# JuliaLinearAlgebra/RecursiveFactorization.jl

Hardware: AMD Instinct MI355X
Metric: LU GFLOP/s (2n^3/3) on NxN Float64, 1/2/4/8 MI355X; ||PA-LU||/||A|| (higher is better)
Workload: dtype f64; 1 GPU; lu!(A, ipiv) of a dense uniform[0,1) 16384x16384 Float64 matrix, partial pivoting, column-major in HBM; n=16384, pivot=True, blocksize=0, layout=single GPU

## Files before the change

recursivefactorization.jl_amd/build.py:

```python
from __future__ import annotations

import os
import subprocess
from concurrent.futures import ThreadPoolExecutor

HERE = os.path.dirname(os.path.abspath(__file__))
CSRC = os.path.join(HERE, "csrc")
OBJ = os.path.join(CSRC, "build_exp" if os.environ.get("RFLU_EXPERIMENTS", "0") not in ("", "0") else "build")
LIB = os.path.join(HERE, "librflu_exp.so" if os.environ.get("RFLU_EXPERIMENTS", "0") not in ("", "0") else "librflu.so")
EXPERIMENTS = os.environ.get("RFLU_EXPERIMENTS", "0") not in ("", "0")
SOURCES = ["gemm.hip", "engine.hip", "panel.hip", "panel_f32.hip", "panel_local.hip", "panel_local_f32.hip", "panel_local_xcd.hip", "panel_local_xcd_f32.hip", "panel_single.hip", "panel_single_f32.hip", "trsm.hip", "trsv.hip", "laswp.hip", "butterfly.hip", "driver.cpp"]
if EXPERIMENTS:
    SOURCES += ["panel_blocked.hip", "panel_blocked_f32.hip"]
HEADERS = ["rflu_internal.hpp", os.path.join("..", "..", "include", "rflu.h")]
ALL_HEADERS = HEADERS + ["panel_common.hpp", "panel_xchg.hpp", "trsm_row.hpp", "gemm_tile.hpp", "laswp_strip.hpp", "engine.hpp", "schedule_plan.hpp"]
_PANEL_H = ["panel_common.hpp", "panel_xchg.hpp", "trsm_row.hpp"]
EXTRA_DEPS = {"gemm.hip": ["gemm_tile.hpp"], "engine.hip": ["gemm_tile.hpp", "laswp_strip.hpp", "engine.hpp"], "driver.cpp": ["engine.hpp", "schedule_plan.hpp"],
              "laswp.hip": ["laswp_strip.hpp", "trsm_row.hpp"], "trsm.hip": ["trsm_row.hpp"], "trsv.hip": ["trsm_row.hpp"],
              "panel.hip": _PANEL_H, "panel_local.hip": _PANEL_H, "panel_single.hip": _PANEL_H, "panel_blocked.hip": _PANEL_H,
              "panel_f32.hip": ["panel.hip", *_PANEL_H], "panel_local_f32.hip": ["panel_local.hip", *_PANEL_H],
              "panel_local_xcd.hip": ["panel_local.hip", *_PANEL_H], "panel_local_xcd_f32.hip": ["panel_local.hip", *_PANEL_H],
              "panel_single_f32.hip": ["panel_single.hip", *_PANEL_H], "panel_blocked_f32.hip": ["panel_blocked.hip", *_PANEL_H]}
FLAGS = ["--offload-arch=gfx950", "-O3", "-std=c++17", "-fPIC", "-x", "hip", "-Wno-unused-result"] + (["-DRFLU_EXPERIMENTS"] if EXPERIMENTS else [])


def _mtime(p):
    return os.path.getmtime(p) if os.path.exists(p) else 0.0


def _digest(paths):
    import hashlib

    h = hashlib.sha1(" ".join(FLAGS).encode())
    for p in paths:
        with open(p, "rb") as f:
            h.update(f.read())
    return h.hexdigest()


def sources_digest() -> str:
# ... 56 lines not shown
```

recursivefactorization.jl_amd/csrc/driver.cpp:

```cpp
#include <stdarg.h>
#include <stdio.h>
#include <stdlib.h>
#include <string.h>

#include <algorithm>
#include <new>

#include "rflu_internal.hpp"
#include "engine.hpp"
#include "schedule_plan.hpp"
#include <atomic>
#include <chrono>
#include <thread>

namespace rflu {

static thread_local char g_err[512] = "";

void set_error(const char* fmt, ...)
{
    va_list ap;
    va_start(ap, fmt);
    vsnprintf(g_err, sizeof(g_err), fmt, ap);
    va_end(ap);
// ... 59 lines not shown
    env_get("RFLU_SPLIT_SHARE", split_share);
    env_get("RFLU_MAX_RESERVE", max_reserve);
    env_get("RFLU_WIDE_NARROW", wide_narrow);
    env_get("RFLU_NARROW_COLS", narrow_cols);
    env_get("RFLU_RESERVE_CUS", min_reserve);
    env_get("RFLU_CONFINE_ROWS", confine_rows);
    env_get("RFLU_MERGE_ROWS", merge_rows);
    env_get("RFLU_SWAP_SU", swap_su);
    env_get("RFLU_SWAP_LATE", swap_late);
    env_get("RFLU_SWAP_ROWS", swap_rows);
    env_get("RFLU_GATE_FOLD", gate_fold);
    env_flag("RFLU_TIME_ENQUEUE", time_enqueue);
    env_get("RFLU_TAIL_OVERLAP", tail_overlap);
    env_get("RFLU_MGPU_TALL_ROWS", mgpu_tall_rows);
    env_get("RFLU_MGPU_SYNC", mgpu_sync);
    env_get("RFLU_ENGINE_POLICY", engine_policy);
    env_get("RFLU_ENGINE_WGS", engine_wgs);
    env_get("RFLU_ENGINE_WC", engine_wc);
    env_get("RFLU_ENGINE_WRITE_THROUGH", engine_write_through);
    env_get("RFLU_ENGINE_LEAF_XCDS", engine_leaf_xcds);
    env_get("RFLU_ENGINE_LEAF_WGS", engine_leaf_wgs);
    env_get("RFLU_ENGINE_HOST_LAG", engine_host_lag);
    env_get("RFLU_ENGINE_SOLVE_RL", engine_solve_rl);
#endif
}

static void load_handle_env(Handle* h)
{
    h->tune.load_env();
    h->coop_launch = false;
    h->panel_local = 2;
    h->panel_single = 1;
    h->panel_blocked = 0;
    h->panel_local_maxg = 64;
    int v = 0;
    env_get("RFLU_COOP_LAUNCH", v);
    h->coop_launch = v != 0;
    env_get("RFLU_PANEL_LOCAL", h->panel_local);
    env_get("RFLU_PANEL_SINGLE", h->panel_single);
    env_get("RFLU_PANEL_BLOCKED", h->panel_blocked);
    if (h->panel_local == 1) h->panel_local_maxg = 32;
#ifdef RFLU_EXPERIMENTS
    env_get("RFLU_PANEL_LOCAL_MAXG", h->panel_local_maxg);
#endif
}

// ... 4 lines not shown
    if (pad > 0 && ld % 512 == 0) ld += pad;
    return ld;
}

int ensure_buffer(void** ptr, size_t* cap, size_t need)
{
    if (*cap >= need) return RFLU_OK;
    if (*ptr) RFLU_HIP(hipFree(*ptr));
    *ptr = nullptr;
    *cap = 0;
    RFLU_HIP(hipMalloc(ptr, need));
    *cap = need;
    return RFLU_OK;
}

int ensure_bookkeeping(Handle* h, int64_t rows)
{
    const int64_t chunks = (rows + NB - 1) / NB + 1;
    if (chunks <= h->pm_chunks) return RFLU_OK;
    if (h->pm_cnt) RFLU_HIP(hipFree(h->pm_cnt));
    if (h->pm_dst) RFLU_HIP(hipFree(h->pm_dst));
    if (h->pm_src) RFLU_HIP(hipFree(h->pm_src));
    if (h->linv) RFLU_HIP(hipFree(h->linv));
    h->linv = nullptr;
    h->pm_cnt = h->pm_dst = h->pm_src = nullptr;
    h->pm_chunks = 0;
    RFLU_HIP(hipMalloc((void**)&h->pm_cnt, (size_t)chunks * sizeof(int)));
    RFLU_HIP(hipMalloc((void**)&h->pm_dst, (size_t)chunks * 2 * NB * sizeof(int)));
    RFLU_HIP(hipMalloc((void**)&h->pm_src, (size_t)chunks * 2 * NB * sizeof(int)));
    RFLU_HIP(hipMalloc(&h->linv, (size_t)chunks * NB * NB * sizeof(double)));
    RFLU_HIP(hipMemset(h->pm_cnt, 0, (size_t)chunks * sizeof(int)));
    h->pm_chunks = chunks;
    return RFLU_OK;
}

constexpr int64_t TRSM_FUSED_MAX = 256;

template <typename T>
static int trsm_rec(Handle* h, int64_t n, int64_t nrhs, const T* L, int64_t ldl, T* B, int64_t ldb, const T* linv)
{
    if (n <= 0 || nrhs <= 0) return RFLU_OK;
    if (linv && n <= TRSM_FUSED_MAX) return launch_trsm_fused<T>(h, n, nrhs, L, ldl, linv, B, ldb);
    if (n <= NB) return launch_trsm_base<T>(h, n, nrhs, L, ldl, B, ldb);
    const int64_t leaves = (n + NB - 1) / NB;
    const int64_t n1 = ((leaves + 1) / 2) * NB;
    RFLU_TRY(trsm_rec<T>(h, n1, nrhs, L, ldl, B, ldb, linv));
    RFLU_TRY(launch_gemm<T>(h, n - n1, nrhs, n1, L + n1 * ldl, ldl, B, ldb, B + n1 * ldb, ldb));
    return trsm_rec<T>(h, n - n1, nrhs, L + n1 * ldl + n1, ldl, B + n1 * ldb, ldb,
                       linv ? linv + (n1 / NB) * NB * NB : nullptr);
}

template <typename T>
static int trsm_public(Handle* h, int64_t n, int64_t nrhs, const T* L, int64_t ldl, T* B, int64_t ldb)
{
// ... 676 lines not shown
            c.lclaim = lk < nleft ? (unsigned long long)lk << 32 : (unsigned long long)ENG_SEQ_DONE << 32;
            c.lprog = (unsigned long long)lk;
            if (nleft > 0 && lk > 0) img->cb[eng_first_cb(geo, eng_pb(geo, cb))].leftdone += 1ull << 32;
            img->remaining += lk < nleft;
        }
        if (h->tune.engine_replay) {
            if (eng_end < nblk) { set_error("RFLU_ENGINE_REPLAY needs the engine to the end"); return RFLU_ERR_ARG; }
            RFLU_TRY(launch_gate_signal(h, h->gate_ptr[0], val(nleaf - 1)));
            if (f.tail) { RFLU_HIP(hipStreamWaitEvent(P, f.tail, 0)); f.tail = nullptr; }
        }
        RFLU_HIP(hipMemcpyAsync(reinterpret_cast<char*>(est) + skip, reinterpret_cast<char*>(img) + skip, bytes - skip, hipMemcpyHostToDevice, P));
        RFLU_TRY(record_on(P, EX + (size_t)nblk + 1));
        RFLU_TRY(wait_on(E, EX + (size_t)nblk + 1));
        EngArgs<T> a;
        a.R = R; a.ld = ld; a.g = geo; a.policy = h->tune.engine_policy;
        a.linv = static_cast<const T*>(h->linv); a.pm_cnt = h->pm_cnt; a.pm_dst = h->pm_dst; a.pm_src = h->pm_src;
        a.st = est; a.leaf_gate = h->gate_ptr[0]; a.gate_base = gbase; a.info = h->info_dev; a.gemm_flags = h->tune.gemm_flags;
        a.arrived = h->eng_host_mode ? &est->arrived : nullptr;
        a.rows_final = h->eng_host_mode ? h->eng_rows_final_dev : nullptr;
        a.write_through = h->tune.engine_write_through != 0;
        a.leaf_xcds = h->tune.engine_leaf_xcds;
        a.leaf_wgs = h->tune.engine_leaf_wgs;
        a.solve_rl = h->tune.engine_solve_rl != 0;
        a.host_lag = h->eng_host_mode ? h->tune.engine_host_lag : 0;
        a.retire_xcc = -1; a.retire_leaf = 0;
        if (eng_retire_leaf >= 0) {
            a.retire_xcc = h->panel_xcc;
            a.retire_leaf = (int)std::max<int64_t>(1, eng_retire_leaf - 2);
        }
        a.trace = nullptr;
        long long*& eng_trace_buf = h->eng_trace_buf;
        if (env_str("RFLU_ENGINE_TRACE")) {
            if (!eng_trace_buf) RFLU_HIP(hipMalloc((void**)&eng_trace_buf, (4096 * 4 + 16) * sizeof(long long)));
            else {
                std::vector<long long> hs(4096 * 4 + 16);
                RFLU_HIP(hipMemcpy(hs.data(), eng_trace_buf, hs.size() * sizeof(long long), hipMemcpyDeviceToHost));
                double s01 = 0, s12 = 0, s23 = 0, sq = 0; int cnt = 0;
                for (int g = 1; g + 1 < (int)nleaf && g < 4095; ++g) {
                    if (!hs[g * 4] || !hs[g * 4 + 3] || !hs[(g - 1) * 4 + 3]) continue;
                    s01 += (hs[g * 4 + 1] - hs[g * 4]) / 100.0; s12 += (hs[g * 4 + 2] - hs[g * 4 + 1]) / 100.0; s23 += (hs[g * 4 + 3] - hs[g * 4 + 2]) / 100.0;
                    sq += (hs[g * 4] - hs[(g - 1) * 4 + 3]) / 100.0; ++cnt;
                }
                if (cnt) fprintf(stderr, "[rflu] engine trace (previous call, %d leaf windows on their first column block): first claim -> stage 0 done %.1f us, -> first tile claimed %.1f, -> window complete %.1f; previous window complete -> first claim %.1f us\n", cnt, s01 / cnt, s12 / cnt, s23 / cnt, sq / cnt);
                {
                    const long long* ac = hs.data() + 4096 * 4;
                    const double tot = (double)(ac[0] + ac[1] + ac[2] + ac[3] + ac[4]);
                    if (tot > 0)
                        fprintf(stderr, "[rflu] engine workgroup time (previous call, %.1f workgroup-ms): block-column tiles %.1f %%, leaf-window tiles %.1f %%, strips + solves %.1f %%, deferred interchanges %.1f %%, between units %.1f %% (of which asleep with nothing eligible %.1f %%, count + publication behind a unit %.1f %%, scan / claim / acquire %.1f %%)\n",
                                tot / 1e5, 100.0 * ac[0] / tot, 100.0 * ac[1] / tot, 100.0 * ac[2] / tot, 100.0 * ac[3] / tot, 100.0 * ac[4] / tot, 100.0 * ac[5] / tot, 100.0 * ac[6] / tot, 100.0 * (ac[4] - ac[5] - ac[6]) / tot);
                    if (tot > 0 && ac[15] > 0)
                        fprintf(stderr, "[rflu] engine scan (previous call, %lld calls, %.2f sweeps per call), us per call: epoch / gate sample %.2f, exit words %.2f, claim words + choice %.2f, ticket %.2f, "
                                        "scan of the deferred interchanges %.2f, acquire + hand-over %.2f; asleep %.2f\n",
                                ac[15], (double)ac[14] / ac[15], ac[8] / 100.0 / ac[15], ac[9] / 100.0 / ac[15], ac[10] / 100.0 / ac[15], ac[11] / 100.0 / ac[15], ac[12] / 100.0 / ac[15],
                                ac[13] / 100.0 / ac[15], ac[5] / 100.0 / ac[15]);
                }
                int tg0 = 40, tgn = 4;
                if (const char* e = env_str("RFLU_ENGINE_TRACE")) { if (strchr(e, ':')) sscanf(e, "%d:%d", &tg0, &tgn); }
                for (int g = std::max(tg0, 1); g < tg0 + tgn && g + 1 < (int)nleaf && g < 4095; ++g)
                {
                    fprintf(stderr, "   leaf %d: first claim at %.3f ms | stage 0 %.1f us | to first tile %.1f | tiles %.1f | idle before %.1f", g, (hs[g * 4] - hs[0]) / 1e5,
                            (hs[g * 4 + 1] - hs[g * 4]) / 100.0, (hs[g * 4 + 2] - hs[g * 4 + 1]) / 100.0, (hs[g * 4 + 3] - hs[g * 4 + 2]) / 100.0, (hs[g * 4] - hs[(g - 1) * 4 + 3]) / 100.0);
                    const long long* n4 = hs.data() + (size_t)(2048 + g) * 4;
                    if (g < 2048 && n4[0] && n4[3])
                        fprintf(stderr, " || next block column: first claim at %.3f ms (%.1f us after the previous leaf's window there was complete) | stage 0 %.1f | to first tile %.1f | tiles %.1f",
                                (n4[0] - hs[0]) / 1e5, (n4[0] - n4[-1]) / 100.0, (n4[1] - n4[0]) / 100.0, (n4[2] - n4[1]) / 100.0, (n4[3] - n4[2]) / 100.0);
                    fprintf(stderr, "\n");
                    const int LPBt = (int)(W / NB);
                    if ((g + 1) % LPBt == 0 && g / LPBt < 512) {
                        const int b = g / LPBt;
                        const long long* bg = hs.data() + (size_t)(1024 + b) * 4;
                        const long long* lf = hs.data() + (size_t)(1536 + b) * 4;
                        const long long t0 = n4[0];
                        if (t0 && bg[0] && bg[3])
                            fprintf(stderr, "   block column %d ends (its last leaf's window is claimed at +0): own deferred interchanges +%.0f .. +%.0f us | BIG(%d) on the first column block of block column %d: "
                                            "stage 0 +%.0f .. +%.0f | tiles +%.0f .. +%.0f us\n",
                                    b, (lf[0] - t0) / 100.0, (lf[1] - t0) / 100.0, b, b + 2, (bg[0] - t0) / 100.0, (bg[1] - t0) / 100.0, (bg[2] - t0) / 100.0, (bg[3] - t0) / 100.0);
                    }
                }
            }
            RFLU_HIP(hipMemsetAsync(eng_trace_buf, 0, (4096 * 4 + 16) * sizeof(long long), P));
            a.trace = eng_trace_buf;
        }
        const int wgs = h->tune.engine_wgs > 0 ? h->tune.engine_wgs : 2 * (h->num_cus - 32);
        if (img->remaining > 0) {
            double eng_flops = 0, eng_bytes = 0;
            for (int cb = 0; cb < geo.ncb; ++cb) {
                for (int k = 0; k < eng_nops(geo, cb); ++k) {
                    const EngOp o = eng_op(geo, cb, k);
                    if (o.nc <= 0) continue;
                    const double M = (double)std::max(geo.m - (o.j0 + o.jb), 0), N = (double)o.nc, K = (double)o.jb;
                    eng_flops += 2.0 * M * N * K;
                    eng_bytes += sizeof(T) * (M * K + K * N + 2.0 * M * N + 2.0 * K * N + 0.5 * K * K + (f.pivot ? 4.0 * K * N : 0.0));
                }
                if (f.pivot && eng_pb(geo, cb) < geo.nbp) {
                    const double nc = (double)(std::min<int64_t>(n, (int64_t)(cb + 1) * geo.Wc) - (int64_t)cb * geo.Wc);
                    const double later = (double)std::max<int64_t>(std::min<int64_t>((int64_t)geo.nbp * W, mn) - (int64_t)(eng_pb(geo, cb) + 1) * W, 0);
                    eng_bytes += sizeof(T) * 4.0 * nc * (0.5 * (double)std::min<int64_t>(W, mn - (int64_t)eng_pb(geo, cb) * W) + later);
                }
            }
            hipStream_t saved = h->stream;
            h->stream = E;
            int rc;
            {
// ... 766 lines not shown
    RFLU_HIP(hipEventCreate(&h->ev1));
    h->panel_max_wgs = panel_resident_limit(h->num_cus);
    if (h->panel_max_wgs <= 0) { set_error("occupancy query for the cooperative panel kernels failed"); delete h; return RFLU_ERR_HIP; }
    load_handle_env(h);
    *handle = reinterpret_cast<rflu_handle_t>(h);
    return RFLU_OK;
}

int rflu_destroy(rflu_handle_t handle)
{
    if (!handle) return RFLU_OK;
    Handle* h = H(handle);
    DeviceGuard device_guard__(h->device);
    (void)hipStreamSynchronize(h->stream);
    if (h->work) (void)hipFree(h->work);
    if (h->ipiv_dev) (void)hipFree(h->ipiv_dev);
    if (h->hostA_dev) (void)hipFree(h->hostA_dev);
    if (h->out_stage) (void)hipFree(h->out_stage);
    if (h->rhs_work) (void)hipFree(h->rhs_work);
    if (h->hostB_dev) (void)hipFree(h->hostB_dev);
    if (h->pm_cnt) (void)hipFree(h->pm_cnt);
    if (h->pm_dst) (void)hipFree(h->pm_dst);
    if (h->pm_src) (void)hipFree(h->pm_src);
    if (h->linv) (void)hipFree(h->linv);
    if (h->linv_tmp) (void)hipFree(h->linv_tmp);
    if (h->pscratch) (void)hipFree(h->pscratch);
    if (h->info_dev) (void)hipFree(h->info_dev);
    if (h->gates) (void)hipFree(h->gates);
    if (h->tail_event_obj) (void)hipEventDestroy(h->tail_event_obj);
    if (h->tail_fork_obj) (void)hipEventDestroy(h->tail_fork_obj);
    if (h->gate_stamps) (void)hipFree(h->gate_stamps);
    if (h->eng_state) (void)hipFree(h->eng_state);
    if (h->eng_host) (void)hipHostFree(h->eng_host);
    if (h->eng_rows_final) (void)hipHostFree(h->eng_rows_final);
    if (h->eng_trace_buf) (void)hipFree(h->eng_trace_buf);
    if (h->info_pinned) (void)hipHostFree(h->info_pinned);
    if (h->ev0) (void)hipEventDestroy(h->ev0);
    if (h->ev1) (void)hipEventDestroy(h->ev1);
    for (hipEvent_t e : h->out_events) (void)hipEventDestroy(e);
    for (void* b : h->bounce) if (b) (void)hipHostFree(b);
    for (hipStream_t ps : h->parked_streams)
        if (ps) (void)hipStreamDestroy(ps);
    if (h->qprobe_slots) (void)hipFree(h->qprobe_slots);
    for (hipStream_t us : h->ustreams)
        if (us) (void)hipStreamDestroy(us);
    for (hipStream_t ps : h->pstreams)
// ... 750 lines not shown
```

recursivefactorization.jl_amd/csrc/engine.hip:

```cpp
#include <limits.h>

#include "engine.hpp"
#include "gemm_tile.hpp"
#include "laswp_strip.hpp"

namespace rflu {

constexpr int EP_COLS = ENG_PREP_COLS;
constexpr int EP_XLD = EP_COLS + 1;

template <typename T>
__device__ __forceinline__ int eng_units(const EngArgs<T>& a, int cb, unsigned seq)
{
    return eng_units_of(eng_op(a.g, cb, (int)(seq >> 1)), (int)(seq & 1u), a.g.m);
}

typedef unsigned long long __attribute__((address_space(1))) EngGWord;
__device__ __forceinline__ unsigned long long eng_load(const unsigned long long* p)
{
    return __hip_atomic_load((const EngGWord*)p, __ATOMIC_RELAXED, __HIP_MEMORY_SCOPE_AGENT);
}
__device__ __forceinline__ void eng_store(unsigned long long* p, unsigned long long v)
{
    __hip_atomic_store((EngGWord*)p, v, __ATOMIC_RELAXED, __HIP_MEMORY_SCOPE_AGENT);
}
__device__ __forceinline__ unsigned long long eng_add(unsigned long long* p, unsigned long long v)
{
    return __hip_atomic_fetch_add((EngGWord*)p, v, __ATOMIC_RELAXED, __HIP_MEMORY_SCOPE_AGENT);
}
__device__ __forceinline__ void eng_max(unsigned long long* p, unsigned long long v)
{
    __hip_atomic_fetch_max((EngGWord*)p, v, __ATOMIC_RELAXED, __HIP_MEMORY_SCOPE_AGENT);
}
__device__ __forceinline__ void eng_release()
{
    __builtin_amdgcn_fence(__ATOMIC_RELEASE, "agent");
    asm volatile("s_waitcnt vmcnt(0)" ::: "memory");
}

template <typename T>
struct EngUnit {
    typedef T __attribute__((address_space(1))) GT;
    typedef int __attribute__((address_space(1))) GI;
    typedef T __attribute__((address_space(3))) LT;
    GT* R;
    const GT* linv;
    const GI* pm_cnt;
    const GI* pm_dst;
    const GI* pm_src;
    LT* smem;
    int64_t ld;
    EngGeo g;
    int gemm_flags;
    int write_through;
    int solve_rl;
};
template <typename T>
__device__ __forceinline__ EngUnit<T> eng_unit_args(const EngArgs<T>& a, T* smem)
{
    EngUnit<T> u;
    u.R = (typename EngUnit<T>::GT*)a.R;
    u.linv = (const typename EngUnit<T>::GT*)a.linv;
    u.pm_cnt = (const typename EngUnit<T>::GI*)a.pm_cnt;
    u.pm_dst = (const typename EngUnit<T>::GI*)a.pm_dst;
    u.pm_src = (const typename EngUnit<T>::GI*)a.pm_src;
    u.smem = (typename EngUnit<T>::LT*)smem;
    u.ld = a.ld;
    u.g = a.g;
    u.gemm_flags = a.gemm_flags;
    u.write_through = a.write_through;
    u.solve_rl = a.solve_rl;
    return u;
}

template <typename T>
__device__ __attribute__((noinline)) void eng_prep_unit(const EngUnit<T> a, const EngOp o, int u)
{
    T* const smem = (T*)a.smem;
    typedef typename Mfma<T>::acc_t acc_t;
    constexpr int VW = 16 / (int)sizeof(T);
    const int tid = threadIdx.x, lane = tid & 63, wave = tid >> 6;
    constexpr bool UNI = sizeof(T) == 8;
    auto uni = [](int v) { return UNI ? __builtin_amdgcn_readfirstlane(v) : v; };
    auto uni64 = [](unsigned long long v) {
        return UNI ? ((unsigned long long)(unsigned)__builtin_amdgcn_readfirstlane((int)(v >> 32)) << 32) | (unsigned long long)(unsigned)__builtin_amdgcn_readfirstlane((int)v) : v;
    };
    const int j0 = uni(o.j0), jb = uni(o.jb);
    const int c0 = uni(o.c_lo + u * EP_COLS);
    const int nc = uni(min(EP_COLS, o.nc - u * EP_COLS));
    T* const R = (T*)uni64((unsigned long long)(T*)a.R);
    const int64_t ld = (int64_t)uni64((unsigned long long)a.ld);
    const int* const pm_cnt = (const int*)a.pm_cnt;
    const int* const pm_dst = (const int*)a.pm_dst;
    const int* const pm_src = (const int*)a.pm_src;
    if (a.g.pivot) {
        const int wv = __builtin_amdgcn_readfirstlane(wave);
        if (nc % VW == 0) {
            constexpr int SC = 8 * VW;
            if (wv < (nc + SC - 1) / SC)
                laswp_strip<T, VW, 8>(R, ld, c0, nc, 0, 0, 0, 0, pm_cnt, pm_dst, pm_src, o.chunk0, o.chunk1, wv);
        } else {
            if (wv < (nc + 7) / 8)
                laswp_strip<T, 1, 8>(R, ld, c0, nc, 0, 0, 0, 0, pm_cnt, pm_dst, pm_src, o.chunk0, o.chunk1, wv);
        }
        __syncthreads();
    }
    const T* L = R + (int64_t)j0 * ld + j0;
    const T* Linv = (const T*)uni64((unsigned long long)(const T*)a.linv) + (int64_t)(j0 / NB) * NB * NB;
    T* B = R + (int64_t)j0 * ld + c0;
    const int nblk = (jb + NB - 1) / NB;
    const int fi = lane & 15, fk = lane >> 4;
    const int arow = wave * 16 + fi;
    T* Xd = smem;
    constexpr int EP_MAXBLK = 8;
    if (nblk <= EP_MAXBLK && a.solve_rl) {
        acc_t acc[EP_MAXBLK][2];
#pragma unroll
        for (int e = 0; e < EP_MAXBLK; ++e) {
            const int rows_e = e < nblk ? min(NB, jb - e * NB) : 0;
#pragma unroll
            for (int t = 0; t < 2; ++t)
#pragma unroll
                for (int r = 0; r < 4; ++r) {
                    const int row = wave * 16 + Mfma<T>::crow(lane, r);
                    const int col = t * 16 + fi;
                    acc[e][t][r] = (row < rows_e && col < nc) ? B[(int64_t)(e * NB + row) * ld + col] : T(0);
                }
        }
        auto load_l = [&](T (&av)[16], int e, int d) {
            const bool rok = arow < min(NB, jb - e * NB);
            const T* Lp = L + (int64_t)(e * NB + arow) * ld + d * NB + 16 * fk;
            if (rok) {
                typedef T ep_vec __attribute__((ext_vector_type(VW)));
#pragma unroll
                for (int v = 0; v < 16 / VW; ++v) {
                    const ep_vec y = *reinterpret_cast<const ep_vec*>(Lp + v * VW);
#pragma unroll
                    for (int q = 0; q < VW; ++q) av[v * VW + q] = -y[q];
                }
            } else {
#pragma unroll
                for (int kk = 0; kk < 16; ++kk) av[kk] = T(0);
            }
        };
        auto load_inv = [&](T (&ai)[16], int d) {
            const T* Ip = Linv + (int64_t)d * NB * NB + arow * NB + 16 * fk;
            typedef T ep_vec __attribute__((ext_vector_type(VW)));
#pragma unroll
            for (int v = 0; v < 16 / VW; ++v) {
                const ep_vec x = *reinterpret_cast<const ep_vec*>(Ip + v * VW);
#pragma unroll
// ... 36 lines not shown
#pragma unroll
                    for (int r = 0; r < 4; ++r) {
                        const int row = wave * 16 + Mfma<T>::crow(lane, r);
                        const int col = t * 16 + fi;
                        const bool in = row < rows_d && col < nc;
                        if (in) B[(int64_t)(d * NB + row) * ld + col] = x[t][r];
                        Xd[row * EP_XLD + col] = in ? x[t][r] : T(0);
                    }
                if (d + 1 < nblk) {
                    __syncthreads();
#pragma unroll
                    for (int e = d + 1; e < EP_MAXBLK; e += 2) {
                        if (e < nblk) {
                            if (e + 1 < nblk) load_l(avB, e + 1, d);
                            mul_l(avA, acc[e]);
                            if (e + 2 < nblk) load_l(avA, e + 2, d);
                            if (e + 1 < nblk) mul_l(avB, acc[e + 1 < EP_MAXBLK ? e + 1 : e]);
                        }
                    }
                    __syncthreads();
                }
            }
        }
        return;
    }
    for (int d = 0; d < nblk; ++d) {
        const int rows_d = min(NB, jb - d * NB);
        acc_t acc[2];
#pragma unroll
        for (int t = 0; t < 2; ++t)
#pragma unroll
            for (int r = 0; r < 4; ++r) {
                const int row = wave * 16 + Mfma<T>::crow(lane, r);
                const int col = t * 16 + fi;
                acc[t][r] = (row < rows_d && col < nc) ? B[(int64_t)(d * NB + row) * ld + col] : T(0);
            }
        const bool rok = arow < rows_d;
        for (int e = 0; e < d; ++e) {
            T av[16], b0[16], b1[16];
            const T* Lp = L + (int64_t)(d * NB + arow) * ld + e * NB + 16 * fk;
            const T* Xe = B + (int64_t)(e * NB + 16 * fk) * ld + fi;
            if (rok) {
                typedef T ep_vec __attribute__((ext_vector_type(VW)));
#pragma unroll
                for (int v = 0; v < 16 / VW; ++v) {
                    const ep_vec x = *reinterpret_cast<const ep_vec*>(Lp + v * VW);
// ... 30 lines not shown
                for (int q = 0; q < VW; ++q) ai[v * VW + q] = x[q];
            }
        }
        __syncthreads();
        acc_t x[2] = {acc_t{T(0), T(0), T(0), T(0)}, acc_t{T(0), T(0), T(0), T(0)}};
#pragma unroll
        for (int kk = 0; kk < 16; ++kk) {
            const T q0 = Xd[(16 * fk + kk) * EP_XLD + fi];
            const T q1 = Xd[(16 * fk + kk) * EP_XLD + 16 + fi];
            x[0] = Mfma<T>::run(ai[kk], q0, x[0]);
            x[1] = Mfma<T>::run(ai[kk], q1, x[1]);
        }
#pragma unroll
        for (int t = 0; t < 2; ++t)
#pragma unroll
            for (int r = 0; r < 4; ++r) {
                const int row = wave * 16 + Mfma<T>::crow(lane, r);
                const int col = t * 16 + fi;
                if (row < rows_d && col < nc) B[(int64_t)(d * NB + row) * ld + col] = x[t][r];
            }
        asm volatile("s_waitcnt vmcnt(0)" ::: "memory");
        __syncthreads();
    }
}

template <typename T>
__device__ __attribute__((noinline)) void eng_gemm_unit(const EngUnit<T> a, const EngOp o, int t)
{
    constexpr int VW = 16 / (int)sizeof(T);
    T* const smem = (T*)a.smem;
    auto uni = [](int v) { return __builtin_amdgcn_readfirstlane(v); };
    auto uni64 = [](unsigned long long v) {
        return ((unsigned long long)(unsigned)__builtin_amdgcn_readfirstlane((int)(v >> 32)) << 32) | (unsigned long long)(unsigned)__builtin_amdgcn_readfirstlane((int)v);
    };
    T* const Rg = (T*)uni64((unsigned long long)(T*)a.R);
    const int64_t ld = (int64_t)uni64((unsigned long long)a.ld);
    const int oj0 = uni(o.j0), ojb = uni(o.jb), oclo = uni(o.c_lo);
    t = uni(t);
    const int je = oj0 + ojb;
    GemmArgs<T> g;
    g.M = uni(a.g.m) - je;
    g.N = uni(o.nc);
    g.K = ojb;
    g.A = Rg + (int64_t)je * ld + oj0;
    g.B = Rg + (int64_t)oj0 * ld + oclo;
    g.C = Rg + (int64_t)je * ld + oclo;
// ... 24 lines not shown

template <typename T>
__device__ __attribute__((noinline)) void eng_left_unit(const EngUnit<T> a, int cb, int lk, int u)
{
    constexpr int VW = 16 / (int)sizeof(T);
    constexpr int SC = 8 * VW;
    const int wave = __builtin_amdgcn_readfirstlane(threadIdx.x >> 6);
    const int LPB = a.g.W / NB;
    const int pb = eng_pb(a.g, cb);
    const int cb0 = cb * a.g.Wc;
    const int ncb_cols = min(a.g.Wc, a.g.n - cb0);
    int c0, nc, chunk0, chunk1;
    if (lk == 0) {
        c0 = cb0 + u * NB;
        nc = min(NB, ncb_cols - u * NB);
        chunk0 = c0 / NB + 1;
        chunk1 = pb * LPB + eng_leaves_of_block(a.g, pb);
    } else {
        c0 = cb0 + u * 4 * SC;
        nc = min(4 * SC, ncb_cols - u * 4 * SC);
        chunk0 = (pb + lk) * LPB;
        chunk1 = chunk0 + eng_leaves_of_block(a.g, pb + lk);
    }
    if (nc <= 0 || chunk1 <= chunk0) return;
    T* const R = (T*)a.R;
    const int* const pm_cnt = (const int*)a.pm_cnt;
    const int* const pm_dst = (const int*)a.pm_dst;
    const int* const pm_src = (const int*)a.pm_src;
    if (nc % VW == 0) {
        for (int s = wave; s < (nc + SC - 1) / SC; s += 4)
            laswp_strip<T, VW, 8>(R, a.ld, c0, nc, 0, 0, 0, 0, pm_cnt, pm_dst, pm_src, chunk0, chunk1, s);
    } else {
        for (int s = wave; s < (nc + 7) / 8; s += 4)
            laswp_strip<T, 1, 8>(R, a.ld, c0, nc, 0, 0, 0, 0, pm_cnt, pm_dst, pm_src, chunk0, chunk1, s);
    }
}

enum { ENG_NONE = 0, ENG_MAIN = 1, ENG_LEFT = 2, ENG_EXIT = 3 };

__shared__ int eng_sel[4];
__shared__ int eng_wst[4];
__shared__ long long eng_nap;
__shared__ long long eng_ph[8];
#define ENG_PH(k) do { if (TRACE && lane == 0) { const long long t_ = wall_clock64(); eng_ph[k] += t_ - ph_t; ph_t = t_; } } while (0)

template <typename T, bool TRACE>
__device__ __attribute__((noinline)) void eng_scan(unsigned long long kernarg)
{
    const unsigned long long ku = ((unsigned long long)(unsigned)__builtin_amdgcn_readfirstlane((unsigned)(kernarg >> 32)) << 32) |
                                  (unsigned long long)(unsigned)__builtin_amdgcn_readfirstlane((unsigned)kernarg);
    EngArgs<T> a;
// ... 347 lines not shown
            if ((seq & 1u) == 0) eng_prep_unit<T>(ua, o, unit);
            else eng_gemm_unit<T>(ua, o, unit);
        } else {
            if (TRACE && tid == 0 && seq == 0 && unit == 0 && cb == eng_first_cb(a.g, eng_pb(a.g, cb)) && eng_pb(a.g, cb) < 512)
                a.trace[(1536 + eng_pb(a.g, cb)) * 4] = wall_clock64();
            eng_left_unit<T>(ua, cb, (int)seq, unit);
        }
        asm volatile("s_waitcnt vmcnt(0)" ::: "memory");
        if (TRACE && tid == 0) { const long long t = wall_clock64(); acct[acct_k] += t - acct_t; acct_t = t; }
        __syncthreads();
        if (tid == 0) eng_complete<T, TRACE>((unsigned long long)__builtin_amdgcn_kernarg_segment_ptr(), kind, cb, seq, unit);
        if (TRACE && tid == 0) acct[6] += wall_clock64() - acct_t;
        __syncthreads();
    }
    if (TRACE && tid == 0) {
        acct[5] = eng_nap;
        for (int k = 0; k < 7; ++k) eng_add((unsigned long long*)&a.trace[4096 * 4 + k], (unsigned long long)acct[k]);
        for (int k = 0; k < 8; ++k) eng_add((unsigned long long*)&a.trace[4096 * 4 + 8 + k], (unsigned long long)eng_ph[k]);
    }
}

size_t engine_lds_bytes(size_t esize)
{
    return std::max<size_t>(2 * (size_t)G_STAGE * esize, (size_t)NB * EP_XLD * esize);
}

template <typename T>
int launch_engine(Handle* h, hipStream_t stream, const EngArgs<T>& a, int wgs)
{
    const size_t lds = engine_lds_bytes(sizeof(T));
    bool& attr_set = h->eng_attr_set[sizeof(T) == 8 ? 0 : 1];
    if (a.trace) {
        RFLU_HIP(hipFuncSetAttribute(reinterpret_cast<const void*>(&engine_kernel<T, true>), hipFuncAttributeMaxDynamicSharedMemorySize, (int)lds));
        hipLaunchKernelGGL((engine_kernel<T, true>), dim3((unsigned)wgs), dim3(256), lds, stream, a);
        RFLU_HIP(hipGetLastError());
        return RFLU_OK;
    }
    if (!attr_set) {
        RFLU_HIP(hipFuncSetAttribute(reinterpret_cast<const void*>(&engine_kernel<T, false>), hipFuncAttributeMaxDynamicSharedMemorySize, (int)lds));
        attr_set = true;
    }
    hipLaunchKernelGGL((engine_kernel<T, false>), dim3((unsigned)wgs), dim3(256), lds, stream, a);
    RFLU_HIP(hipGetLastError());
    return RFLU_OK;
}

template int launch_engine<double>(Handle*, hipStream_t, const EngArgs<double>&, int);
// ... 49 lines not shown
```

recursivefactorization.jl_amd/csrc/engine.hpp:

```cpp
#pragma once

#include <stdint.h>

#include "rflu_internal.hpp"

#if defined(__HIPCC__)
#define RFLU_HD __host__ __device__ __forceinline__
#else
#define RFLU_HD inline
#endif

namespace rflu {

constexpr int ENG_MAX_CB = 512;
constexpr unsigned ENG_SEQ_DONE = 0x7fffffffu;
constexpr int ENG_PREP_COLS = 32;

struct EngCB {
    unsigned long long claim;
    unsigned long long done;
    unsigned long long lclaim;
    unsigned long long ldone;
    unsigned long long prog;
    unsigned long long leftdone;
    unsigned long long lprog;
    unsigned long long bigdone;
};
// ... 163 lines not shown

template <typename T>
struct EngArgs {
    T* R;
    int64_t ld;
    EngGeo g;
    int policy;
    const T* linv;
    const int* pm_cnt;
    const int* pm_dst;
    const int* pm_src;
    EngState* st;
    const unsigned long long* leaf_gate;
    unsigned long long gate_base;
    int64_t* info;
    const unsigned long long* arrived;
    unsigned long long* rows_final;
    int gemm_flags;
    long long* trace;
    int write_through;
    int leaf_xcds;
    int leaf_wgs;
    int solve_rl;
    int host_lag;
    int retire_xcc;
    int retire_leaf;
};

template <typename T>
int launch_engine(Handle* h, hipStream_t stream, const EngArgs<T>& a, int wgs);
int launch_eng_wait(Handle* h, const unsigned long long* flag, unsigned long long value);
int launch_eng_wait_retired(Handle* h, int xcc);
size_t engine_lds_bytes(size_t esize);

}
```

recursivefactorization.jl_amd/csrc/rflu_internal.hpp:

```cpp
#pragma once

#include <hip/hip_runtime.h>
#include <stdint.h>

#include <functional>
#include <vector>

#include "../../include/rflu.h"

namespace rflu {

constexpr int NB = 64;
constexpr int PANEL_THREADS = 512;
constexpr int MAX_PANEL_WGS = 256;

void set_error(const char* fmt, ...);
#define RFLU_HIP(call)                                                                         \
    do {                                                                                       \
        hipError_t e__ = (call);                                                               \
        if (e__ != hipSuccess) {                                                               \
            ::rflu::set_error("%s failed: %s (%s:%d)", #call, hipGetErrorString(e__), __FILE__, __LINE__); \
            return RFLU_ERR_HIP;                                                               \
        }                                                                                      \
    } while (0)
// ... 55 lines not shown
    int64_t host_early_out = 512;
    int host_trace = 0;
    int swap_late = 1;
    int64_t swap_rows = 8192;
    int leaf_fuse = 1;
    int host_threads = 8;
    int64_t mgpu_big_reserve = 128;
    int64_t mgpu_tall_rows = -1;
    int mgpu_sync = 0;
    int debug_ghost_leaf = -1;
    int engine = -1;
    int engine_policy = 0;
    int engine_wgs = 0;
    int64_t engine_rows = 0;
    int engine_wc = 512;
    int engine_retire = -1;
    int engine_replay = 0;
    int engine_host = 1;
    int engine_write_through = 1;
    int engine_leaf_xcds = 1;
    int engine_leaf_wgs = 16;
    int engine_ahead = 1;
    int engine_solve_rl = 1;
    int engine_host_lag = 5;
    void load_env();
};

struct Handle {
    Tune tune;
    int device = 0;
    hipStream_t own_stream = nullptr;
    hipStream_t stream = nullptr;
    hipStream_t ustreams[8] = {};
    bool mask_failed = false;
    std::function<int(int64_t)> progress;
    std::function<int()> before_sync;
    bool out_done = false;
    std::vector<hipEvent_t> out_events;
    void* bounce[2] = {};
    void* out_stage = nullptr;
    size_t out_stage_bytes = 0;
    size_t bounce_bytes = 0;
    std::vector<hipStream_t> parked_streams;
    long long* qprobe_slots = nullptr;
    std::vector<hipStream_t> queues_ok_streams;
    int queues_ok_count = 0;
// ... 6 lines not shown
    unsigned long long* gates = nullptr;
    unsigned long long* gate_ptr[3] = {};
    unsigned long long gate_epoch = 0;
    long long* gate_stamps = nullptr;
    std::vector<hipEvent_t> events;
    int last_path = RFLU_PATH_NONE;
    int num_cus = 256;

    void* work = nullptr;
    size_t work_bytes = 0;
    int64_t* ipiv_dev = nullptr;
    size_t ipiv_cap = 0;
    void* hostA_dev = nullptr;
    size_t hostA_bytes = 0;
    void* rhs_work = nullptr;
    size_t rhs_work_bytes = 0;
    void* hostB_dev = nullptr;
    size_t hostB_bytes = 0;

    int* pm_cnt = nullptr;
    int* pm_dst = nullptr;
    int* pm_src = nullptr;
    int64_t pm_chunks = 0;
    void* linv = nullptr;
    unsigned trsv_tag = 0;
    void* trsv_area = nullptr;
    void* linv_tmp = nullptr;
    size_t linv_tmp_bytes = 0;

    unsigned long long* pscratch = nullptr;
    size_t pscratch_bytes = 0;
    unsigned epoch = 1;
    int coop_leaf_seq = 0;
    int64_t* info_dev = nullptr;
    int panel_local = 2;
    int panel_single = 1;
    int panel_blocked = 0;
    int panel_local_maxg = 64;
    int panel_xcc = 0;
    int64_t local_rows_cap = -1;
    int trsv_max_wgs[2] = {0, 0};
    int trsm32_per_cu[2] = {0, 0};
    int trsm16_per_cu[2] = {0, 0};
    int panel_max_wgs = 0;
    bool coop_launch = false;
    bool la_attr_set[2] = {false, false};
// ... 144 lines not shown
```

Before: 41790 GFLOP/s.

## Compose deferred row interchanges and gather pivoted rows during the engine prep solve

```diff
diff --git a/recursivefactorization.jl_amd/build.py b/recursivefactorization.jl_amd/build.py
--- a/recursivefactorization.jl_amd/build.py
+++ b/recursivefactorization.jl_amd/build.py
@@ -13,9 +13,9 @@
 if EXPERIMENTS:
     SOURCES += ["panel_blocked.hip", "panel_blocked_f32.hip"]
 HEADERS = ["rflu_internal.hpp", os.path.join("..", "..", "include", "rflu.h")]
-ALL_HEADERS = HEADERS + ["panel_common.hpp", "panel_xchg.hpp", "trsm_row.hpp", "gemm_tile.hpp", "laswp_strip.hpp", "engine.hpp", "schedule_plan.hpp"]
+ALL_HEADERS = HEADERS + ["panel_common.hpp", "panel_xchg.hpp", "trsm_row.hpp", "gemm_tile.hpp", "laswp_strip.hpp", "engine.hpp", "schedule_plan.hpp", "perm_compose.hpp"]
 _PANEL_H = ["panel_common.hpp", "panel_xchg.hpp", "trsm_row.hpp"]
-EXTRA_DEPS = {"gemm.hip": ["gemm_tile.hpp"], "engine.hip": ["gemm_tile.hpp", "laswp_strip.hpp", "engine.hpp"], "driver.cpp": ["engine.hpp", "schedule_plan.hpp"],
+EXTRA_DEPS = {"gemm.hip": ["gemm_tile.hpp"], "engine.hip": ["gemm_tile.hpp", "laswp_strip.hpp", "engine.hpp", "perm_compose.hpp"], "driver.cpp": ["engine.hpp", "schedule_plan.hpp", "perm_compose.hpp"],
               "laswp.hip": ["laswp_strip.hpp", "trsm_row.hpp"], "trsm.hip": ["trsm_row.hpp"], "trsv.hip": ["trsm_row.hpp"],
               "panel.hip": _PANEL_H, "panel_local.hip": _PANEL_H, "panel_single.hip": _PANEL_H, "panel_blocked.hip": _PANEL_H,
               "panel_f32.hip": ["panel.hip", *_PANEL_H], "panel_local_f32.hip": ["panel_local.hip", *_PANEL_H],
diff --git a/recursivefactorization.jl_amd/csrc/driver.cpp b/recursivefactorization.jl_amd/csrc/driver.cpp
--- a/recursivefactorization.jl_amd/csrc/driver.cpp
+++ b/recursivefactorization.jl_amd/csrc/driver.cpp
@@ -105,6 +105,7 @@
     env_get("RFLU_ENGINE_LEAF_WGS", engine_leaf_wgs);
     env_get("RFLU_ENGINE_HOST_LAG", engine_host_lag);
     env_get("RFLU_ENGINE_SOLVE_RL", engine_solve_rl);
+    env_get("RFLU_ENGINE_GATHER", engine_gather);
 #endif
 }
 
@@ -155,14 +156,24 @@
     if (h->pm_dst) RFLU_HIP(hipFree(h->pm_dst));
     if (h->pm_src) RFLU_HIP(hipFree(h->pm_src));
     if (h->linv) RFLU_HIP(hipFree(h->linv));
+    if (h->cp_top) RFLU_HIP(hipFree(h->cp_top));
+    if (h->cp_bdst) RFLU_HIP(hipFree(h->cp_bdst));
+    if (h->cp_bsrc) RFLU_HIP(hipFree(h->cp_bsrc));
+    if (h->cp_cnt) RFLU_HIP(hipFree(h->cp_cnt));
     h->linv = nullptr;
     h->pm_cnt = h->pm_dst = h->pm_src = nullptr;
+    h->cp_top = h->cp_bdst = h->cp_bsrc = h->cp_cnt = nullptr;
     h->pm_chunks = 0;
     RFLU_HIP(hipMalloc((void**)&h->pm_cnt, (size_t)chunks * sizeof(int)));
     RFLU_HIP(hipMalloc((void**)&h->pm_dst, (size_t)chunks * 2 * NB * sizeof(int)));
     RFLU_HIP(hipMalloc((void**)&h->pm_src, (size_t)chunks * 2 * NB * sizeof(int)));
     RFLU_HIP(hipMalloc(&h->linv, (size_t)chunks * NB * NB * sizeof(double)));
+    RFLU_HIP(hipMalloc((void**)&h->cp_top, (size_t)chunks * NB * sizeof(int)));
+    RFLU_HIP(hipMalloc((void**)&h->cp_bdst, (size_t)chunks * NB * sizeof(int)));
+    RFLU_HIP(hipMalloc((void**)&h->cp_bsrc, (size_t)chunks * NB * sizeof(int)));
+    RFLU_HIP(hipMalloc((void**)&h->cp_cnt, (size_t)chunks * sizeof(int)));
     RFLU_HIP(hipMemset(h->pm_cnt, 0, (size_t)chunks * sizeof(int)));
+    RFLU_HIP(hipMemset(h->cp_cnt, 0, (size_t)chunks * sizeof(int)));
     h->pm_chunks = chunks;
     return RFLU_OK;
 }
@@ -885,6 +896,9 @@
         a.leaf_xcds = h->tune.engine_leaf_xcds;
         a.leaf_wgs = h->tune.engine_leaf_wgs;
         a.solve_rl = h->tune.engine_solve_rl != 0;
+        a.cp_top = h->cp_top; a.cp_bdst = h->cp_bdst; a.cp_bsrc = h->cp_bsrc; a.cp_cnt = h->cp_cnt;
+        a.gather = h->tune.engine_gather != 0;
+        if (geo.pivot && m > PC_MAX_ROWS) { set_error("factor_leafwise: the engine composes the interchanges of at most 16384 rows"); return RFLU_ERR_ARG; }
         a.host_lag = h->eng_host_mode ? h->tune.engine_host_lag : 0;
         a.retire_xcc = -1; a.retire_leaf = 0;
         if (eng_retire_leaf >= 0) {
@@ -894,9 +908,9 @@
         a.trace = nullptr;
         long long*& eng_trace_buf = h->eng_trace_buf;
         if (env_str("RFLU_ENGINE_TRACE")) {
-            if (!eng_trace_buf) RFLU_HIP(hipMalloc((void**)&eng_trace_buf, (4096 * 4 + 16) * sizeof(long long)));
+            if (!eng_trace_buf) RFLU_HIP(hipMalloc((void**)&eng_trace_buf, (4096 * 4 + 16 + 512) * sizeof(long long)));
             else {
-                std::vector<long long> hs(4096 * 4 + 16);
+                std::vector<long long> hs(4096 * 4 + 16 + 512);
                 RFLU_HIP(hipMemcpy(hs.data(), eng_trace_buf, hs.size() * sizeof(long long), hipMemcpyDeviceToHost));
                 double s01 = 0, s12 = 0, s23 = 0, sq = 0; int cnt = 0;
                 for (int g = 1; g + 1 < (int)nleaf && g < 4095; ++g) {
@@ -936,12 +950,14 @@
                         const long long t0 = n4[0];
                         if (t0 && bg[0] && bg[3])
                             fprintf(stderr, "   block column %d ends (its last leaf's window is claimed at +0): own deferred interchanges +%.0f .. +%.0f us | BIG(%d) on the first column block of block column %d: "
-                                            "stage 0 +%.0f .. +%.0f | tiles +%.0f .. +%.0f us\n",
-                                    b, (lf[0] - t0) / 100.0, (lf[1] - t0) / 100.0, b, b + 2, (bg[0] - t0) / 100.0, (bg[1] - t0) / 100.0, (bg[2] - t0) / 100.0, (bg[3] - t0) / 100.0);
+                                            "stage 0 +%.0f .. +%.0f (gather + displaced rows %.0f us, solve %.0f us) | tiles +%.0f .. +%.0f us\n",
+                                    b, (lf[0] - t0) / 100.0, (lf[1] - t0) / 100.0, b, b + 2, (bg[0] - t0) / 100.0, (bg[1] - t0) / 100.0,
+                                    hs[4096 * 4 + 16 + b] ? (hs[4096 * 4 + 16 + b] - bg[0]) / 100.0 : 0.0, hs[4096 * 4 + 16 + b] ? (bg[1] - hs[4096 * 4 + 16 + b]) / 100.0 : (bg[1] - bg[0]) / 100.0,
+                                    (bg[2] - t0) / 100.0, (bg[3] - t0) / 100.0);
                     }
                 }
             }
-            RFLU_HIP(hipMemsetAsync(eng_trace_buf, 0, (4096 * 4 + 16) * sizeof(long long), P));
+            RFLU_HIP(hipMemsetAsync(eng_trace_buf, 0, (4096 * 4 + 16 + 512) * sizeof(long long), P));
             a.trace = eng_trace_buf;
         }
         const int wgs = h->tune.engine_wgs > 0 ? h->tune.engine_wgs : 2 * (h->num_cus - 32);
@@ -1754,6 +1770,10 @@
     if (h->pm_cnt) (void)hipFree(h->pm_cnt);
     if (h->pm_dst) (void)hipFree(h->pm_dst);
     if (h->pm_src) (void)hipFree(h->pm_src);
+    if (h->cp_top) (void)hipFree(h->cp_top);
+    if (h->cp_bdst) (void)hipFree(h->cp_bdst);
+    if (h->cp_bsrc) (void)hipFree(h->cp_bsrc);
+    if (h->cp_cnt) (void)hipFree(h->cp_cnt);
     if (h->linv) (void)hipFree(h->linv);
     if (h->linv_tmp) (void)hipFree(h->linv_tmp);
     if (h->pscratch) (void)hipFree(h->pscratch);
diff --git a/recursivefactorization.jl_amd/csrc/engine.hip b/recursivefactorization.jl_amd/csrc/engine.hip
--- a/recursivefactorization.jl_amd/csrc/engine.hip
+++ b/recursivefactorization.jl_amd/csrc/engine.hip
@@ -7,6 +7,9 @@
 namespace rflu {
 
 constexpr int EP_COLS = ENG_PREP_COLS;
+#ifndef RFLU_ENG_PREP_PRIO
+#define RFLU_ENG_PREP_PRIO 0
+#endif
 constexpr int EP_XLD = EP_COLS + 1;
 
 template <typename T>
@@ -48,12 +51,18 @@
     const GI* pm_cnt;
     const GI* pm_dst;
     const GI* pm_src;
+    GI* cp_top;
+    GI* cp_bdst;
+    GI* cp_bsrc;
+    GI* cp_cnt;
+    long long __attribute__((address_space(1)))* trace;
     LT* smem;
     int64_t ld;
     EngGeo g;
     int gemm_flags;
     int write_through;
     int solve_rl;
+    int gather;
 };
 template <typename T>
 __device__ __forceinline__ EngUnit<T> eng_unit_args(const EngArgs<T>& a, T* smem)
@@ -70,8 +79,16 @@
     u.gemm_flags = a.gemm_flags;
     u.write_through = a.write_through;
     u.solve_rl = a.solve_rl;
+    u.gather = a.gather;
+    u.trace = (long long __attribute__((address_space(1)))*)a.trace;
+    u.cp_top = (typename EngUnit<T>::GI*)a.cp_top;
+    u.cp_bdst = (typename EngUnit<T>::GI*)a.cp_bdst;
+    u.cp_bsrc = (typename EngUnit<T>::GI*)a.cp_bsrc;
+    u.cp_cnt = (typename EngUnit<T>::GI*)a.cp_cnt;
     return u;
 }
+
+__shared__ int eng_pc_cnt;
 
 template <typename T>
 __device__ __attribute__((noinline)) void eng_prep_unit(const EngUnit<T> a, const EngOp o, int u)
@@ -80,6 +97,7 @@
     typedef typename Mfma<T>::acc_t acc_t;
     constexpr int VW = 16 / (int)sizeof(T);
     const int tid = threadIdx.x, lane = tid & 63, wave = tid >> 6;
+    if (RFLU_ENG_PREP_PRIO) __builtin_amdgcn_s_setprio(RFLU_ENG_PREP_PRIO);
     constexpr bool UNI = sizeof(T) == 8;
     auto uni = [](int v) { return UNI ? __builtin_amdgcn_readfirstlane(v) : v; };
     auto uni64 = [](unsigned long long v) {
@@ -93,7 +111,10 @@
     const int* const pm_cnt = (const int*)a.pm_cnt;
     const int* const pm_dst = (const int*)a.pm_dst;
     const int* const pm_src = (const int*)a.pm_src;
-    if (a.g.pivot) {
+    constexpr int EP_MAXBLK = 8;
+    const int nblk = (jb + NB - 1) / NB;
+    const bool gather = a.g.pivot && a.gather && nc % VW == 0 && nblk <= EP_MAXBLK && a.solve_rl;
+    if (a.g.pivot && !gather) {
         const int wv = __builtin_amdgcn_readfirstlane(wave);
         if (nc % VW == 0) {
             constexpr int SC = 8 * VW;
@@ -108,25 +129,81 @@
     const T* L = R + (int64_t)j0 * ld + j0;
     const T* Linv = (const T*)uni64((unsigned long long)(const T*)a.linv) + (int64_t)(j0 / NB) * NB * NB;
     T* B = R + (int64_t)j0 * ld + c0;
-    const int nblk = (jb + NB - 1) / NB;
     const int fi = lane & 15, fk = lane >> 4;
     const int arow = wave * 16 + fi;
     T* Xd = smem;
-    constexpr int EP_MAXBLK = 8;
     if (nblk <= EP_MAXBLK && a.solve_rl) {
+        typedef int __attribute__((address_space(3))) LI;
+        int* const tsrc = (int*)((LI*)(a.smem + NB * EP_XLD));
+        int* const bdst = tsrc + EP_MAXBLK * NB;
+        int* const bsrc = bdst + EP_MAXBLK * NB;
+        int nbel = 0;
+        if (gather) {
+            if (o.chunk1 - o.chunk0 > 1) {
+                const int* const cp_top = (const int*)a.cp_top;
+                const int* const cp_bdst = (const int*)a.cp_bdst;
+                const int* const cp_bsrc = (const int*)a.cp_bsrc;
+                nbel = min(jb, __builtin_amdgcn_readfirstlane(__hip_atomic_load((const int*)a.cp_cnt + o.chunk0, __ATOMIC_RELAXED, __HIP_MEMORY_SCOPE_AGENT)));
+                for (int i = tid; i < jb; i += 256) tsrc[i] = cp_top[j0 + i];
+                for (int i = tid; i < nbel; i += 256) { bdst[i] = cp_bdst[j0 + i]; bsrc[i] = cp_bsrc[j0 + i]; }
+                __syncthreads();
+            } else {
+                const int cnt = min(2 * NB, __builtin_amdgcn_readfirstlane(__hip_atomic_load(pm_cnt + o.chunk0, __ATOMIC_RELAXED, __HIP_MEMORY_SCOPE_AGENT)));
+                int ms = 0, md = 0;
+                if (tid < cnt) { ms = pm_src[(size_t)o.chunk0 * 2 * NB + tid]; md = pm_dst[(size_t)o.chunk0 * 2 * NB + tid]; }
+                if (tid < jb) tsrc[tid] = j0 + tid;
+                if (tid == 0) eng_pc_cnt = 0;
+                __syncthreads();
+                if (tid < cnt) {
+                    if (pc_dst_is_top(j0, jb, md)) tsrc[md - j0] = ms;
+                    else {
+                        const int k = atomicAdd(&eng_pc_cnt, 1);
+                        if (k < EP_MAXBLK * NB) { bdst[k] = md; bsrc[k] = ms; }
+                    }
+                }
+                __syncthreads();
+                nbel = min(EP_MAXBLK * NB, __builtin_amdgcn_readfirstlane(eng_pc_cnt));
+            }
+        }
         acc_t acc[EP_MAXBLK][2];
 #pragma unroll
         for (int e = 0; e < EP_MAXBLK; ++e) {
             const int rows_e = e < nblk ? min(NB, jb - e * NB) : 0;
 #pragma unroll
-            for (int t = 0; t < 2; ++t)
-#pragma unroll
-                for (int r = 0; r < 4; ++r) {
-                    const int row = wave * 16 + Mfma<T>::crow(lane, r);
+            for (int r = 0; r < 4; ++r) {
+                const int row = wave * 16 + Mfma<T>::crow(lane, r);
+                const bool rin = row < rows_e;
+                const int srow = (gather && rin) ? tsrc[e * NB + row] : j0 + e * NB + row;
+#pragma unroll
+                for (int t = 0; t < 2; ++t) {
                     const int col = t * 16 + fi;
-                    acc[e][t][r] = (row < rows_e && col < nc) ? B[(int64_t)(e * NB + row) * ld + col] : T(0);
-                }
-        }
+                    acc[e][t][r] = (rin && col < nc) ? R[(int64_t)srow * ld + c0 + col] : T(0);
+                }
+            }
+        }
+        if (gather) {
+            asm volatile("s_waitcnt vmcnt(0)" ::: "memory");
+            __syncthreads();
+            typedef T ep_vec __attribute__((ext_vector_type(VW)));
+            constexpr int LPR = EP_COLS / VW, RPW = 64 / LPR;
+            constexpr int BATCH = 32 / RPW;
+            const int cl = (lane % LPR) * VW, rs = lane / LPR;
+            for (int base = 0; base < nbel; base += 4 * RPW * BATCH) {
+                ep_vec v[BATCH];
+#pragma unroll
+                for (int i = 0; i < BATCH; ++i) {
+                    const int k = base + (i * 4 + wave) * RPW + rs;
+                    if (k < nbel && cl < nc) v[i] = *reinterpret_cast<const ep_vec*>(R + (int64_t)bsrc[k] * ld + c0 + cl);
+                }
+#pragma unroll
+                for (int i = 0; i < BATCH; ++i) {
+                    const int k = base + (i * 4 + wave) * RPW + rs;
+                    if (k < nbel && cl < nc) *reinterpret_cast<ep_vec*>(R + (int64_t)bdst[k] * ld + c0 + cl) = v[i];
+                }
+            }
+        }
+        if (a.trace && tid == 0 && u == 0 && o.type == ENG_OP_BIG && j0 / a.g.W < 512 && o.c_lo == eng_first_cb(a.g, j0 / a.g.W + eng_ahead(a.g) + 1) * a.g.Wc)
+            a.trace[4096 * 4 + 16 + j0 / a.g.W] = wall_clock64();
         auto load_l = [&](T (&av)[16], int e, int d) {
             const bool rok = arow < min(NB, jb - e * NB);
             const T* Lp = L + (int64_t)(e * NB + arow) * ld + d * NB + 16 * fk;
@@ -209,6 +286,7 @@
                 }
             }
         }
+        if (RFLU_ENG_PREP_PRIO) __builtin_amdgcn_s_setprio(0);
         return;
     }
     for (int d = 0; d < nblk; ++d) {
@@ -285,6 +363,7 @@
         asm volatile("s_waitcnt vmcnt(0)" ::: "memory");
         __syncthreads();
     }
+    if (RFLU_ENG_PREP_PRIO) __builtin_amdgcn_s_setprio(0);
 }
 
 template <typename T>
@@ -355,11 +434,56 @@
         chunk0 = (pb + lk) * LPB;
         chunk1 = chunk0 + eng_leaves_of_block(a.g, pb + lk);
     }
-    if (nc <= 0 || chunk1 <= chunk0) return;
-    T* const R = (T*)a.R;
     const int* const pm_cnt = (const int*)a.pm_cnt;
     const int* const pm_dst = (const int*)a.pm_dst;
     const int* const pm_src = (const int*)a.pm_src;
+    if (lk == 0 && nc > 0 && chunk1 == chunk0 && a.gather) {
+        const int tid = threadIdx.x;
+        const int j0 = pb * a.g.W;
+        const int jb = min(a.g.W, a.g.mn - j0);
+        const int rows = min(a.g.m - j0, PC_MAX_ROWS);
+        const int c_first = pb * LPB;
+        constexpr int CP_MAXCH = 8;
+        typedef pc_map_t __attribute__((address_space(3))) LM;
+        pc_map_t* const orig = (pc_map_t*)((LM*)a.smem);
+        int cnt[CP_MAXCH], ms[CP_MAXCH], md[CP_MAXCH];
+#pragma unroll
+        for (int t = 0; t < CP_MAXCH; ++t) {
+            cnt[t] = 0; ms[t] = md[t] = j0;
+            if (c_first + t < chunk1) {
+                cnt[t] = min(2 * NB, __hip_atomic_load(pm_cnt + c_first + t, __ATOMIC_RELAXED, __HIP_MEMORY_SCOPE_AGENT));
+                if (tid < cnt[t]) { ms[t] = pm_src[(size_t)(c_first + t) * 2 * NB + tid]; md[t] = pm_dst[(size_t)(c_first + t) * 2 * NB + tid]; }
+            }
+        }
+        for (int p = tid; p < rows; p += 256) pc_init(orig, p);
+        if (tid == 0) eng_pc_cnt = 0;
+        __syncthreads();
+#pragma unroll
+        for (int t = 0; t < CP_MAXCH; ++t) {
+            if (c_first + t < chunk1) {
+                const bool mine = tid < cnt[t] && ms[t] >= j0 && md[t] >= j0 && ms[t] - j0 < rows && md[t] - j0 < rows;
+                int v = 0;
+                if (mine) v = pc_move_read(orig, j0, ms[t]);
+                __syncthreads();
+                if (mine) pc_move_write(orig, j0, md[t], v);
+                __syncthreads();
+            }
+        }
+        int* const cp_top = (int*)a.cp_top;
+        int* const cp_bdst = (int*)a.cp_bdst;
+        int* const cp_bsrc = (int*)a.cp_bsrc;
+        for (int i = tid; i < jb; i += 256) cp_top[j0 + i] = pc_top_src(orig, j0, i);
+        for (int p = jb + tid; p < rows; p += 256)
+            if (pc_below_moved(orig, p)) {
+                const int k = atomicAdd(&eng_pc_cnt, 1);
+                if (k < jb) { cp_bdst[j0 + k] = j0 + p; cp_bsrc[j0 + k] = pc_below_src(orig, j0, p); }
+            }
+        __syncthreads();
+        if (tid == 0) ((int*)a.cp_cnt)[c_first] = min(eng_pc_cnt, jb);
+        return;
+    }
+    if (nc <= 0 || chunk1 <= chunk0) return;
+    T* const R = (T*)a.R;
     if (nc % VW == 0) {
         for (int s = wave; s < (nc + SC - 1) / SC; s += 4)
             laswp_strip<T, VW, 8>(R, a.ld, c0, nc, 0, 0, 0, 0, pm_cnt, pm_dst, pm_src, chunk0, chunk1, s);
@@ -753,7 +877,7 @@
 
 size_t engine_lds_bytes(size_t esize)
 {
-    return std::max<size_t>(2 * (size_t)G_STAGE * esize, (size_t)NB * EP_XLD * esize);
+    return std::max<size_t>(std::max<size_t>(2 * (size_t)G_STAGE * esize, (size_t)NB * EP_XLD * esize + 3 * 8 * NB * sizeof(int)), (size_t)PC_MAX_ROWS * sizeof(pc_map_t));
 }
 
 template <typename T>
diff --git a/recursivefactorization.jl_amd/csrc/engine.hpp b/recursivefactorization.jl_amd/csrc/engine.hpp
--- a/recursivefactorization.jl_amd/csrc/engine.hpp
+++ b/recursivefactorization.jl_amd/csrc/engine.hpp
@@ -3,6 +3,7 @@
 #include <stdint.h>
 
 #include "rflu_internal.hpp"
+#include "perm_compose.hpp"
 
 #if defined(__HIPCC__)
 #define RFLU_HD __host__ __device__ __forceinline__
@@ -212,6 +213,11 @@
     int leaf_xcds;
     int leaf_wgs;
     int solve_rl;
+    int gather;
+    int* cp_top;
+    int* cp_bdst;
+    int* cp_bsrc;
+    int* cp_cnt;
     int host_lag;
     int retire_xcc;
     int retire_leaf;
diff --git a/recursivefactorization.jl_amd/csrc/perm_compose.hpp b/recursivefactorization.jl_amd/csrc/perm_compose.hpp
--- /dev/null
+++ b/recursivefactorization.jl_amd/csrc/perm_compose.hpp
@@ -0,0 +1,31 @@
+#pragma once
+
+#include <stdint.h>
+
+#if defined(__HIPCC__)
+#include <hip/hip_runtime.h>
+#endif
+
+#ifndef RFLU_HD
+#if defined(__HIPCC__)
+#define RFLU_HD __host__ __device__ __forceinline__
+#else
+#define RFLU_HD inline
+#endif
+#endif
+
+namespace rflu {
+
+constexpr int PC_MAX_ROWS = 16384;
+typedef unsigned short pc_map_t;
+
+RFLU_HD void pc_init(pc_map_t* orig, int p) { orig[p] = (pc_map_t)p; }
+RFLU_HD int pc_move_read(const pc_map_t* orig, int j0, int src) { return (int)orig[src - j0]; }
+RFLU_HD void pc_move_write(pc_map_t* orig, int j0, int dst, int v) { orig[dst - j0] = (pc_map_t)v; }
+RFLU_HD int pc_top_src(const pc_map_t* orig, int j0, int i) { return j0 + (int)orig[i]; }
+RFLU_HD bool pc_below_moved(const pc_map_t* orig, int p) { return (int)orig[p] != p; }
+RFLU_HD int pc_below_src(const pc_map_t* orig, int j0, int p) { return j0 + (int)orig[p]; }
+
+RFLU_HD bool pc_dst_is_top(int j0, int jb, int dst) { return dst < j0 + jb; }
+
+}
diff --git a/recursivefactorization.jl_amd/csrc/rflu_internal.hpp b/recursivefactorization.jl_amd/csrc/rflu_internal.hpp
--- a/recursivefactorization.jl_amd/csrc/rflu_internal.hpp
+++ b/recursivefactorization.jl_amd/csrc/rflu_internal.hpp
@@ -101,6 +101,7 @@
     int engine_leaf_wgs = 16;
     int engine_ahead = 1;
     int engine_solve_rl = 1;
+    int engine_gather = 1;
     int engine_host_lag = 5;
     void load_env();
 };
@@ -153,6 +154,10 @@
     int* pm_dst = nullptr;
     int* pm_src = nullptr;
     int64_t pm_chunks = 0;
+    int* cp_top = nullptr;
+    int* cp_bdst = nullptr;
+    int* cp_bsrc = nullptr;
+    int* cp_cnt = nullptr;
     void* linv = nullptr;
     unsigned trsv_tag = 0;
     void* trsv_area = nullptr;
```

Result: no change. 41770 GFLOP/s (-0.0%).
